# penghao-wu/vstar

Hardware: AMD Instinct MI355X
Metric: searched crops/sec (336x336 tiles, 7B VSM bf16) (higher is better)
Workload: dtype bf16; 1 GPU; BASELINE config 2: 32-crop batches/GPU, CLIP-ViT-L/14@336 (P=576) + LLaMA-7B prefill S=640 + OWL-ViT-B/16@768 + det/SAM heads, records all-gathered per step; seq_len=640, parallelism=dp1

## Files before the change

### include/vstar_hip.h

```cpp
#ifndef VSTAR_HIP_H
#define VSTAR_HIP_H

#include <stdint.h>
#include <stddef.h>

#ifdef __cplusplus
extern "C" {
#endif

#define VSTAR_ABI_VERSION 1

enum { VSTAR_F32 = 0, VSTAR_F16 = 1, VSTAR_BF16 = 2 };

enum {
  VSTAR_OK = 0,
  VSTAR_ERR_INVALID = -1,
  VSTAR_ERR_STATE = -2,
  VSTAR_ERR_MISSING = -3,
  VSTAR_ERR_HIP = -4,
  VSTAR_ERR_NOMEM = -5
};

typedef struct vstar_config {
  int32_t abi_version;
// ... 96 lines not shown
       VSTAR_EPI_NOSYNC = 0x100,
       VSTAR_EPI_TILE128 = 0x200,
       VSTAR_EPI_TILE256 = 0x400,
       VSTAR_EPI_TILE4W = 0x800    };

int vstar_op_gemm(void* stream, const uint16_t* dev_A, int64_t lda, const uint16_t* dev_W, const uint16_t* dev_bias,
                  const uint16_t* dev_residual, int64_t ldr, void* dev_C, int64_t ldc, int out_f32,
                  int M, int N, int K, int epilogue);
int vstar_op_gemm_norm(void* stream, const uint16_t* dev_A, int64_t lda, const uint16_t* dev_W, const uint16_t* dev_bias,
                       const uint16_t* dev_residual, int64_t ldr, void* dev_C, int64_t ldc, int M, int N, int K, int epilogue,
                       const float* dev_row_scale, float* dev_sumsq_out, int sumsq_ld);
int vstar_op_rms_rstd(void* stream, const uint16_t* dev_x, const float* dev_partials, int ld, int rows, int cols, float eps,
                      float* dev_r);
int vstar_op_ln_fold(void* stream, uint16_t* dev_W, uint16_t* dev_bias, const uint16_t* dev_g, const uint16_t* dev_b_ln,
                     int n_rows, int K);
int vstar_op_gemm_last_tile(void);
int vstar_op_gemm_plan(int M, int N, int K, int epilogue, int has_residual, int fused_rope, int cus);
int vstar_op_gemm_fp8(void* stream, const uint16_t* dev_A, const uint16_t* dev_W, const uint16_t* dev_bias,
                      const uint16_t* dev_residual, uint16_t* dev_C, int M, int N, int K, int epilogue, int iters, float* gemm_ms);
size_t vstar_op_mx_scale_bytes(int rows, int cols);
int64_t vstar_op_mx_scale_offset(int row, int k_block, int rows);
int vstar_op_quantize_mx(void* stream, const uint16_t* dev_X, uint8_t* dev_q, uint8_t* dev_scales, int rows, int cols);
int vstar_op_gemm_mx(void* stream, const uint8_t* dev_Aq, const uint8_t* dev_a_scales, const float* dev_row_scale, const uint16_t* dev_W,
                     const uint16_t* dev_residual, uint16_t* dev_C, uint8_t* dev_C8, uint8_t* dev_c_scales, float* dev_sumsq, int M, int N, int K,
                     int epilogue, int iters, float* gemm_ms);
int vstar_op_gemm_fp8_mxout(void* stream, const uint16_t* dev_A, const uint16_t* dev_W, uint8_t* dev_C8, uint8_t* dev_c_scales, int M, int N,
                            int K, int iters, float* gemm_ms);
int vstar_op_attention_mx(void* stream, const uint16_t* dev_qkv, uint8_t* dev_out8, uint8_t* dev_scales, int B, int S, int H);
int vstar_w8a8_mx_active(vstar_handle* h);
int vstar_op_layernorm(void* stream, const uint16_t* dev_x, const uint16_t* dev_gamma, const uint16_t* dev_beta,
// ... 47 lines not shown
```

### vstar_amd/_lib.py

```python
from __future__ import annotations

import ctypes
import os
from ctypes import POINTER, c_char_p, c_double, c_float, c_int, c_int32, c_int64, c_size_t, c_uint, c_uint16, c_void_p

from .config import CVqaConfig, CVstarConfig, MASK_RES, MAX_VERIFY, N_BOXES

LIB_PATH = os.environ.get("VSTAR_LIB") or os.path.join(os.path.dirname(os.path.abspath(__file__)), "libvstar_hip.so")

EXPORTS = [
    "vstar_create", "vstar_destroy", "vstar_last_error", "vstar_load_tensor", "vstar_finalize_weights",
    "vstar_vsm_score_batch", "vstar_upsample_mask", "vstar_debug_read", "vstar_stream", "vstar_profile_enable",
    "vstar_profile_read", "vstar_profile_read_fp8", "vstar_op_gemm", "vstar_op_layernorm", "vstar_op_rmsnorm", "vstar_op_attention",
    "vstar_op_attention_workspace", "vstar_image_set", "vstar_preprocess_crops", "vstar_heatmap_stats", "vstar_heatmap_stats_batch", "vstar_vsm_generate", "vstar_op_gemm_fp8",
    "vstar_op_gemm_last_tile", "vstar_op_gemm_plan", "vstar_op_gemm_norm", "vstar_op_rms_rstd", "vstar_op_ln_fold", "vstar_upsample_mask_ex", "vstar_vsm_score_grouped",
    "vstar_image_set_slot", "vstar_image_set_slot_async", "vstar_preprocess_crops_slots", "vstar_comm_unique_id", "vstar_comm_init", "vstar_allgather_results",
    "vstar_comm_destroy", "vstar_build_source_hash", "vstar_op_mx_scale_bytes", "vstar_op_mx_scale_offset", "vstar_op_quantize_mx",
    "vstar_op_gemm_mx", "vstar_op_gemm_fp8_mxout", "vstar_op_attention_mx", "vstar_w8a8_mx_active",
    "vstar_op_owl_class_logits", "vstar_op_owl_box_finish", "vstar_op_upsample2x_im2col3x3", "vstar_op_hyper_mask",
    "vstar_op_im2col_patch", "vstar_op_vit_assemble_tokens", "vstar_op_llm_embed_text", "vstar_op_add_bcast",
    "vstar_op_add_bcast_repeat", "vstar_op_bcast_rows", "vstar_op_owl_cls_mul", "vstar_op_gather_rows", "vstar_op_argmax_rows",
    "vstar_op_layernorm_ex", "vstar_op_rmsnorm_ex", "vstar_op_ln_rstd", "vstar_op_scale_cols", "vstar_op_fill",
    "vstar_op_quantize_rows_fp8", "vstar_op_rmsnorm_quant_fp8", "vstar_op_small_attention",
]

EXPORTS_VQA = [
    "vstar_vqa_create", "vstar_vqa_destroy", "vstar_vqa_last_error", "vstar_vqa_load_tensor", "vstar_vqa_finalize_weights",
    "vstar_vqa_encode_images", "vstar_vqa_forward", "vstar_vqa_debug_read", "vstar_vqa_last_forward_ms", "vstar_vqa_op_gemm",
    "vstar_vqa_forward_sample", "vstar_vqa_op_sample", "vstar_vqa_forward_beam", "vstar_vqa_kv_reorder", "vstar_vqa_kv_copy",
    "vstar_vqa_op_beam_select", "vstar_vqa_forward_score", "vstar_vqa_op_score",
# ... 105 lines not shown
    lib.vstar_profile_enable.restype = c_int
    lib.vstar_profile_read.argtypes = [H, POINTER(c_double), POINTER(c_int64), POINTER(c_double)]
    lib.vstar_profile_read.restype = c_int
    lib.vstar_profile_read_fp8.argtypes = [H, POINTER(c_double), POINTER(c_int64), POINTER(c_double)]
    lib.vstar_profile_read_fp8.restype = c_int
    lib.vstar_op_gemm.argtypes = [c_void_p, c_void_p, c_int64, c_void_p, c_void_p, c_void_p, c_int64, c_void_p, c_int64,
                                  c_int, c_int, c_int, c_int, c_int]
    lib.vstar_op_gemm.restype = c_int
    lib.vstar_op_gemm_norm.argtypes = [c_void_p, c_void_p, c_int64, c_void_p, c_void_p, c_void_p, c_int64, c_void_p, c_int64, c_int, c_int, c_int,
                                       c_int, c_void_p, c_void_p, c_int]
    lib.vstar_op_gemm_norm.restype = c_int
    lib.vstar_op_rms_rstd.argtypes = [c_void_p, c_void_p, c_void_p, c_int, c_int, c_int, c_float, c_void_p]
    lib.vstar_op_rms_rstd.restype = c_int
    lib.vstar_op_ln_fold.argtypes = [c_void_p, c_void_p, c_void_p, c_void_p, c_void_p, c_int, c_int]
    lib.vstar_op_ln_fold.restype = c_int
    lib.vstar_op_gemm_last_tile.argtypes = []
    lib.vstar_op_gemm_last_tile.restype = c_int
    lib.vstar_op_gemm_plan.argtypes = [c_int] * 7
    lib.vstar_op_gemm_plan.restype = c_int
    lib.vstar_op_gemm_fp8.argtypes = [c_void_p, c_void_p, c_void_p, c_void_p, c_void_p, c_void_p, c_int, c_int, c_int, c_int, c_int,
                                      POINTER(c_float)]
    lib.vstar_op_gemm_fp8.restype = c_int
    lib.vstar_op_mx_scale_bytes.argtypes = [c_int, c_int]
    lib.vstar_op_mx_scale_bytes.restype = c_size_t
    lib.vstar_op_mx_scale_offset.argtypes = [c_int, c_int, c_int]
    lib.vstar_op_mx_scale_offset.restype = ctypes.c_int64
    lib.vstar_op_quantize_mx.argtypes = [c_void_p, c_void_p, c_void_p, c_void_p, c_int, c_int]
    lib.vstar_op_quantize_mx.restype = c_int
    lib.vstar_op_gemm_mx.argtypes = [c_void_p] * 10 + [c_int, c_int, c_int, c_int, c_int, POINTER(c_float)]
    lib.vstar_op_gemm_mx.restype = c_int
# ... 111 lines not shown
```

### vstar_amd/csrc/engine.hip

```cpp
#include "llm_cached.hpp"
#include "mx.hpp"
#include <atomic>
#include <tuple>
#include <cstring>

namespace {
struct SamAttn { Lin q, k, v, out; int internal; };
struct SamLayer { SamAttn self_attn, t2i, i2t; lp_t *n1g, *n1b, *n2g, *n2b, *n3g, *n3b, *n4g, *n4b; Lin lin1, lin2; };
}

struct vstar_engine : EngineBase {
  vstar_config cfg{};
  VitTower clip, owl;
  Lin projector;
  lp_t* embed = nullptr;
  std::vector<LlmBlock> llm;
  lp_t* final_norm = nullptr;
  Lin lm_head;
  lp_t* rope = nullptr;
  Lin det0, det1, seg0, seg1;
  lp_t *owl_post_g = nullptr, *owl_post_b = nullptr, *owl_ln_g = nullptr, *owl_ln_b = nullptr;
  Lin cls_fused, box0, box1, box2;
  Lin vis_proj;
  lp_t *no_mask = nullptr, *dense_pe = nullptr, *iou_token = nullptr, *mask_tokens = nullptr;
// ... 17 lines not shown
  float *lr = nullptr, *lpart = nullptr;
  lp_t *lx = nullptr, *lh = nullptr, *lqkv = nullptr, *latt = nullptr, *lact = nullptr;
  lp_t* hsel = nullptr;
  lp_t *sel_att = nullptr, *sel_x = nullptr, *sel_h = nullptr, *sel_act = nullptr;
  float* vlogits = nullptr;
  lp_t *fc_tmp = nullptr, *emb_det = nullptr, *emb_seg = nullptr;
  int32_t *d_ids = nullptr, *d_rowidx = nullptr, *d_argmax = nullptr;
  lp_t *d_clip_pix = nullptr, *d_owl_pix = nullptr;
  lp_t *owl_feats_pre = nullptr, *owl_feats = nullptr, *box_t0 = nullptr, *box_t1 = nullptr;
  float *cls_emb = nullptr, *box_raw = nullptr;
  lp_t *s_src = nullptr, *s_keys = nullptr, *s_kpe = nullptr, *s_ia = nullptr, *s_ib = nullptr, *s_ic = nullptr;
  lp_t *s_tok0 = nullptr, *s_q = nullptr, *s_qpe = nullptr, *s_ta = nullptr, *s_tb = nullptr, *s_tc = nullptr, *s_td = nullptr,
         *s_mlp = nullptr;
  lp_t *s_col1 = nullptr, *s_c1 = nullptr, *s_c1n = nullptr, *s_col2 = nullptr, *s_c2 = nullptr, *s_hyp_in = nullptr,
         *s_hyp_a = nullptr, *s_hyp_b = nullptr, *s_hyper = nullptr;
  int32_t* d_tokidx = nullptr;
  vstar_result* d_results = nullptr;
  int last_B = 0, last_S = 0;
  void* d_stats = nullptr;
  void* d_stats_batch = nullptr; size_t stats_batch_cap = 0;
  void* comm = nullptr;
  float* d_up = nullptr; size_t up_cap = 0;
  struct ImageSlot { uint8_t* d = nullptr; size_t cap = 0; int H = 0, W = 0; };
  ImageSlot images[VSTAR_MAX_IMAGE_SLOTS];
  hipStream_t stream_up = nullptr;
  hipEvent_t ev_up[VSTAR_MAX_IMAGE_SLOTS] = {};
  std::atomic<int> up_pending[VSTAR_MAX_IMAGE_SLOTS] = {};
  uint8_t* h_stage[2] = {nullptr, nullptr};
  size_t stage_cap[2] = {0, 0};
  hipEvent_t ev_stage[2] = {nullptr, nullptr};
// ... 256 lines not shown
  RC(make_lin({"model.mask_decoder.output_upscaling.3.conv.weight"}, {"model.mask_decoder.output_upscaling.3.conv.bias"},
              &conv2, 64 * 9, nullptr, true));
  RC(make_lin({"model.mask_decoder.output_hypernetworks_mlps.0.layers.0.weight"},
              {"model.mask_decoder.output_hypernetworks_mlps.0.layers.0.bias"}, &hyp0, 256));
  RC(make_lin({"model.mask_decoder.output_hypernetworks_mlps.0.layers.1.weight"},
              {"model.mask_decoder.output_hypernetworks_mlps.0.layers.1.bias"}, &hyp1, 256));
  RC(make_lin({"model.mask_decoder.output_hypernetworks_mlps.0.layers.2.weight"},
              {"model.mask_decoder.output_hypernetworks_mlps.0.layers.2.bias"}, &hyp2, 256));
  if (conv1.N != 64 || conv2.N != 32 || hyp2.N != 32) { set_error("mask decoder dims"); return VSTAR_ERR_INVALID; }
  RC(dalloc(&s_src, prow * 256)); RC(dalloc(&s_keys, prow * 256)); RC(dalloc(&s_kpe, prow * 256));
  RC(dalloc(&s_ia, prow * 256)); RC(dalloc(&s_ib, prow * 256)); RC(dalloc(&s_ic, prow * 256));
  const size_t trow = (size_t)maxB * 6;
  RC(dalloc(&s_tok0, trow * 256)); RC(dalloc(&s_q, trow * 256)); RC(dalloc(&s_qpe, trow * 256));
  RC(dalloc(&s_ta, trow * 256)); RC(dalloc(&s_tb, trow * 256)); RC(dalloc(&s_tc, trow * 256)); RC(dalloc(&s_td, trow * 256));
  RC(dalloc(&s_mlp, trow * 2048));
  RC(dalloc(&s_col1, (size_t)maxB * 96 * 96 * 2304));
  RC(dalloc(&s_c1, (size_t)maxB * 96 * 96 * 64));
  RC(dalloc(&s_c1n, (size_t)maxB * 96 * 96 * 64));
  RC(dalloc(&s_col2, (size_t)maxB * 192 * 192 * 576));
  RC(dalloc(&s_c2, (size_t)maxB * 192 * 192 * 32));
  RC(dalloc(&s_hyp_in, (size_t)maxB * 256)); RC(dalloc(&s_hyp_a, (size_t)maxB * 256)); RC(dalloc(&s_hyp_b, (size_t)maxB * 256));
  RC(dalloc(&s_hyper, (size_t)maxB * 32));
  RC(dalloc(&d_tokidx, (size_t)maxB));
  {
    std::vector<int32_t> tix(maxB);
    for (int b = 0; b < maxB; ++b) tix[b] = b * 6 + 1;
    HIPCHK(hipMemcpy(d_tokidx, tix.data(), (size_t)maxB * 4, hipMemcpyHostToDevice));
  }
  RC(dalloc(&d_jobs, (size_t)maxB * 2));
  RC(dalloc(&d_lut, (size_t)3 * 256));
  {
    lp_t lut[3 * 256];
    clip_norm_lut(lut);
    HIPCHK(hipMemcpy(d_lut, lut, sizeof(lut), hipMemcpyHostToDevice));
  }
// ... 394 lines not shown
    RC(lin(s_q, 256, Ly.lin1, s_mlp, Ly.lin1.N, trow, VSTAR_EPI_RELU));
    RC(lin(s_mlp, Ly.lin1.N, Ly.lin2, s_tb, 256, trow, VSTAR_EPI_NONE, s_q, 256));
    KCHK(layernorm_lp(s_tb, Ly.n3g, Ly.n3b, s_q, trow, 256, 1e-5f, nullptr, 0, stream));
    KCHK(add_bcast(s_q, s_tok0, s_qpe, trow, 256, trow, stream));
    RC(sam_attn(Ly.i2t, s_kpe, NP, s_qpe, s_q, T, B, s_ia, s_ta, s_tb, s_ib, s_ic, s_keys));
    KCHK(layernorm_lp(s_ic, Ly.n4g, Ly.n4b, s_keys, prow, 256, 1e-5f, nullptr, 0, stream));
  }
  KCHK(add_bcast(s_q, s_tok0, s_qpe, trow, 256, trow, stream));
  KCHK(add_bcast(s_keys, dense_pe, s_kpe, prow, 256, NP, stream));
  RC(sam_attn(sam_final, s_qpe, T, s_kpe, s_keys, NP, B, s_ta, s_ia, s_ib, s_td, s_tb, s_q));
  KCHK(layernorm_lp(s_tb, sam_nfg, sam_nfb, s_q, trow, 256, 1e-5f, nullptr, 0, stream));
  KCHK(gather_rows(s_q, d_tokidx, s_hyp_in, B, 256, stream));
  RC(lin(s_hyp_in, 256, hyp0, s_hyp_a, 256, B, VSTAR_EPI_RELU));
  RC(lin(s_hyp_a, 256, hyp1, s_hyp_b, 256, B, VSTAR_EPI_RELU));
  RC(lin(s_hyp_b, 256, hyp2, s_hyper, 32, B));
  KCHK(upsample2x_im2col3x3(s_keys, s_col1, B, 48, 48, 256, stream));
  RC(lin(s_col1, 2304, conv1, s_c1, 64, B * 96 * 96));
  KCHK(layernorm_lp(s_c1, ln2d_g, ln2d_b, s_c1n, B * 96 * 96, 64, 1e-6f, nullptr, 1, stream));
  KCHK(upsample2x_im2col3x3(s_c1n, s_col2, B, 96, 96, 64, stream));
  RC(lin(s_col2, 576, conv2, s_c2, 32, B * 192 * 192, VSTAR_EPI_GELU));
  KCHK(hyper_mask(s_hyper, s_c2, res_f + offsetof(vstar_result, lowres_mask) / 4, rstride, B, 192 * 192, 32, stream));
  return 0;
}

int vstar_engine::finish_records(int nrec, int n_verify, unsigned flags, vstar_result* out) {
  if (n_verify > 0) {
    HIPCHK(hipMemcpy2DAsync((char*)d_results + offsetof(vstar_result, tf_argmax), sizeof(vstar_result), d_argmax,
                            (size_t)n_verify * 4, (size_t)n_verify * 4, nrec, hipMemcpyDeviceToDevice, stream));
  }
  if (out) {
    HIPCHK(hipMemcpyAsync(out, d_results, sizeof(vstar_result) * nrec,
                          (flags & VSTAR_F_DEVICE_OUTPUT) ? hipMemcpyDeviceToDevice : hipMemcpyDeviceToHost, stream));
  }
  if (!(flags & VSTAR_F_NO_SYNC)) {
    HIPCHK(hipStreamSynchronize(stream));
    collect_profile();
// ... 287 lines not shown
int vstar_create(const vstar_config* cfg, int device, vstar_handle** out) {
  if (!cfg || !out) { tls_error() = "null argument"; return VSTAR_ERR_INVALID; }
  if (cfg->abi_version != VSTAR_ABI_VERSION) { tls_error() = "ABI version mismatch"; return VSTAR_ERR_INVALID; }
  if (cfg->max_batch <= 0 || cfg->max_text_len < 2) { tls_error() = "bad limits"; return VSTAR_ERR_INVALID; }
  int n = 0;
  hipError_t e = hipGetDeviceCount(&n);
  if (e != hipSuccess || device < 0 || device >= n) {
    tls_error() = "no such HIP device (libvstar_hip has no CPU fallback)";
    return VSTAR_ERR_HIP;
  }
  vstar_engine* h = new vstar_engine();
  h->cfg = *cfg;
  if (const char* e = getenv("VSTAR_FUSED_ROPE")) h->fused_rope = atoi(e) != 0;
  if (const char* e = getenv("VSTAR_FOLD_NORMS")) h->fold_norms = atoi(e) != 0;
  if (const char* e = getenv("VSTAR_SCORE_GRAPH")) h->score_graph_on = atoi(e) != 0;
  h->device = device;
  if (hipSetDevice(device) != hipSuccess || hipStreamCreate(&h->stream) != hipSuccess) {
    tls_error() = "hipStreamCreate failed";
    delete h;
    return VSTAR_ERR_HIP;
  }
  if (const char* e = getenv("VSTAR_OWL_OVERLAP")) h->owl_overlap = atoi(e) != 0;
  if (hipStreamCreate(&h->stream2) != hipSuccess || hipEventCreateWithFlags(&h->ev_fork, hipEventDisableTiming) != hipSuccess ||
      hipEventCreateWithFlags(&h->ev_join, hipEventDisableTiming) != hipSuccess) {
    h->stream2 = nullptr;
  }
  if (hipStreamCreateWithFlags(&h->stream_up, hipStreamNonBlocking) != hipSuccess ||
      hipEventCreateWithFlags(&h->ev_stage[0], hipEventDisableTiming) != hipSuccess ||
      hipEventCreateWithFlags(&h->ev_stage[1], hipEventDisableTiming) != hipSuccess ||
      hipEventCreateWithFlags(&h->ev_pre, hipEventDisableTiming) != hipSuccess) {
// ... 217 lines not shown
  else if (n == "owl_pixels") { src = h->d_owl_pix; cnt = (int64_t)B * 3 * h->cfg.owl_image_size * h->cfg.owl_image_size; }
  else if (n == "clip_features") { src = h->clip.x; cnt = (int64_t)B * h->clip.N * h->clip.hidden; }
  else if (n == "llm_input") { src = h->lx; cnt = 0; }
  else if (n == "llm_hidden_loc") { src = h->hsel; cnt = (int64_t)B * h->cfg.llm_hidden; }
  else if (n == "embed_det") { src = h->emb_det; cnt = (int64_t)B * h->det1.N; }
  else if (n == "embed_seg") { src = h->emb_seg; cnt = (int64_t)B * 256; }
  else if (n == "owl_feats") { src = h->owl_feats; cnt = (int64_t)B * h->owl.P * h->owl.hidden; }
  else if (n == "sam_tokens") { src = h->s_q; cnt = (int64_t)B * 6 * 256; }
  else if (n == "sam_keys") { src = h->s_keys; cnt = (int64_t)B * h->owl.P * 256; }
  else if (n == "sam_src") { src = h->s_src; cnt = (int64_t)B * h->owl.P * 256; }
  else if (n == "sam_c1") { src = h->s_c1; cnt = (int64_t)B * 96 * 96 * 64; }
  else if (n == "sam_c1n") { src = h->s_c1n; cnt = (int64_t)B * 96 * 96 * 64; }
  else if (n == "sam_c2") { src = h->s_c2; cnt = (int64_t)B * 192 * 192 * 32; }
  else if (n == "sam_hyper") { src = h->s_hyper; cnt = (int64_t)B * 32; }
  else { h->set_error("unknown debug tensor: " + n); return VSTAR_ERR_INVALID; }
  if (cnt > cap) cnt = cap;
  std::vector<lp_t> tmp((size_t)cnt);
  if (hipStreamSynchronize(h->stream) != hipSuccess ||
      hipMemcpy(tmp.data(), src, (size_t)cnt * 2, hipMemcpyDeviceToHost) != hipSuccess) {
    h->set_error("debug_read: HIP failure");
    return VSTAR_ERR_HIP;
  }
  for (int64_t i = 0; i < cnt; ++i) out[i] = lp2f(tmp[(size_t)i]);
  return cnt;
}

void* vstar_stream(vstar_handle* h) { return h ? (void*)h->stream : nullptr; }

int vstar_profile_enable(vstar_handle* h, int on) {
  if (!h) return VSTAR_ERR_INVALID;
// ... 251 lines not shown

static int op_done(hipError_t e, void* stream) {
  if (e == hipSuccess) e = hipStreamSynchronize((hipStream_t)stream);
  return op_rc(e);
}
int vstar_op_owl_class_logits(void* stream, const float* emb, int ld, int Q, const uint16_t* query, float* out, int out_stride_crop,
                              int B, int rows_per_crop, int img_div) {
  return op_done(owl_class_logits(emb, ld, Q, query, out, out_stride_crop, B, rows_per_crop, (hipStream_t)stream, img_div), stream);
}
int vstar_op_owl_box_finish(void* stream, const float* raw, int ld, float* out, int out_stride_crop, int B, int grid, int img_div) {
  return op_done(owl_box_finish(raw, ld, out, out_stride_crop, B, grid, (hipStream_t)stream, img_div), stream);
}
int vstar_op_upsample2x_im2col3x3(void* stream, const uint16_t* src, uint16_t* A, int B, int h, int w, int C) {
  return op_done(upsample2x_im2col3x3(src, A, B, h, w, C, (hipStream_t)stream), stream);
}
int vstar_op_hyper_mask(void* stream, const uint16_t* hyper, const uint16_t* up, float* out, int out_stride_crop, int B, int npix,
                        int C) {
  return op_done(hyper_mask(hyper, up, out, out_stride_crop, B, npix, C, (hipStream_t)stream), stream);
}
int vstar_op_im2col_patch(void* stream, const uint16_t* pix, uint16_t* A, int B, int I, int ps, int Kpad) {
  return op_done(im2col_patch(pix, A, B, I, ps, Kpad, (hipStream_t)stream), stream);
}
int vstar_op_vit_assemble_tokens(void* stream, const uint16_t* patch, const uint16_t* cls, const uint16_t* pos, uint16_t* tokens,
                                 int B, int P, int C) {
  return op_done(vit_assemble_tokens(patch, cls, pos, tokens, B, P, C, (hipStream_t)stream), stream);
}
int vstar_op_llm_embed_text(void* stream, const int32_t* ids, int L, int img_col, int P, const uint16_t* table, int vocab,
                            uint16_t* x, int B, int C) {
  return op_done(llm_embed_text(ids, L, img_col, P, table, vocab, x, B, C, (hipStream_t)stream), stream);
}
// ... 58 lines not shown
```

### vstar_amd/csrc/heads.hip

```cpp
#include "common.hpp"
#include "kernels.hpp"

namespace VS_NS {

namespace {

__global__ __launch_bounds__(256) void owl_class_kernel(const float* __restrict__ emb, int ld, int Q,
                                                        const lp_t* __restrict__ query, float* __restrict__ out,
                                                        int out_stride_crop, int B, int rows_per_crop, int img_div) {
  const int lane = threadIdx.x & 63;
  const int64_t row = (int64_t)blockIdx.x * 4 + (threadIdx.x >> 6);
  if (row >= (int64_t)B * rows_per_crop) return;
  const int b = (int)(row / rows_per_crop), p = (int)(row % rows_per_crop);
  const float* er = emb + ((int64_t)(b / img_div) * rows_per_crop + p) * ld;
  const lp_t* qr = query + (int64_t)b * Q;
  float ee = 0.f, qq = 0.f;
  for (int d = lane; d < Q; d += 64) {
    const float e = rlp(er[d]), q = lp2f(qr[d]);
    ee += e * e;
    qq += q * q;
  }
  ee = wave_sum(ee);
  qq = wave_sum(qq);
  const float en = rlp(rlp(sqrtf(ee)) + 1e-6f), qn = rlp(rlp(sqrtf(qq)) + 1e-6f);
// ... 15 lines not shown
  const int64_t idx = (int64_t)blockIdx.x * blockDim.x + threadIdx.x;
  if (idx >= (int64_t)B * npatch * 4) return;
  const int c = (int)(idx & 3);
  const int64_t row = idx >> 2;
  const int p = (int)(row % npatch), b = (int)(row / npatch);
  float coord;
  if (c == 0) coord = (float)(p % grid + 1) / (float)grid;
  else if (c == 1) coord = (float)(p / grid + 1) / (float)grid;
  else coord = 1.0f / (float)grid;
  coord = fminf(fmaxf(coord, 0.f), 1.f);
  const float bias = logf(coord + 1e-4f) - log1pf(-coord + 1e-4f);
  const float v = rlp(rlp(raw[((int64_t)(b / img_div) * npatch + p) * ld + c]) + bias);
  out[(int64_t)b * out_stride_crop + p * 4 + c] = rlp(1.0f / (1.0f + __expf(-v)));
}

__global__ void up2x_im2col_kernel(const lp_t* __restrict__ src, lp_t* __restrict__ A, int B, int h, int w, int C) {
  const int cv = C >> 3;
  const int H2 = 2 * h, W2 = 2 * w;
  const int64_t idx = (int64_t)blockIdx.x * blockDim.x + threadIdx.x;
  const int64_t total = (int64_t)B * H2 * W2 * 9 * cv;
  if (idx >= total) return;
  const int v = (int)(idx % cv);
  int64_t r = idx / cv;
  const int tap = (int)(r % 9);
  r /= 9;
  const int X = (int)(r % W2);
  const int Y = (int)((r / W2) % H2);
  const int b = (int)(r / ((int64_t)W2 * H2));
  const int yy = Y + tap / 3 - 1, xx = X + tap % 3 - 1;
  lpx8 o = {0, 0, 0, 0, 0, 0, 0, 0};
  if (yy >= 0 && yy < H2 && xx >= 0 && xx < W2) {
    const float sy = fmaxf(0.5f * (yy + 0.5f) - 0.5f, 0.f), sx = fmaxf(0.5f * (xx + 0.5f) - 0.5f, 0.f);
    const int y0 = (int)sy, x0 = (int)sx;
    const int y1 = y0 + (y0 < h - 1 ? 1 : 0), x1 = x0 + (x0 < w - 1 ? 1 : 0);
    const float ly = sy - y0, lx = sx - x0;
    const lp_t* base = src + (int64_t)b * h * w * C + v * 8;
    const lpx8 v00 = *(const lpx8*)(base + ((int64_t)y0 * w + x0) * C);
    const lpx8 v01 = *(const lpx8*)(base + ((int64_t)y0 * w + x1) * C);
    const lpx8 v10 = *(const lpx8*)(base + ((int64_t)y1 * w + x0) * C);
    const lpx8 v11 = *(const lpx8*)(base + ((int64_t)y1 * w + x1) * C);
#pragma unroll
    for (int e = 0; e < 8; ++e) {
      const float t = (1.f - ly) * ((1.f - lx) * lp2f((lp_t)v00[e]) + lx * lp2f((lp_t)v01[e])) +
                      ly * ((1.f - lx) * lp2f((lp_t)v10[e]) + lx * lp2f((lp_t)v11[e]));
      o[e] = (short)f2lp(t);
    }
  }
  *(lpx8*)(A + idx * 8) = o;
}

template <int C>
__global__ void hyper_mask_kernel(const lp_t* __restrict__ hyper, const lp_t* __restrict__ up, float* __restrict__ out,
                                  int out_stride_crop, int B, int npix) {
  const int64_t idx = (int64_t)blockIdx.x * blockDim.x + threadIdx.x;
  if (idx >= (int64_t)B * npix) return;
  const int b = (int)(idx / npix), pix = (int)(idx % npix);
  const lp_t* u = up + idx * C;
  const lp_t* hy = hyper + (int64_t)b * C;
  float a = 0.f;
#pragma unroll
  for (int v = 0; v < C / 8; ++v) {
    const lpx8 x = *(const lpx8*)(u + v * 8);
    const lpx8 w = *(const lpx8*)(hy + v * 8);
#pragma unroll
    for (int e = 0; e < 8; ++e) a += lp2f((lp_t)x[e]) * lp2f((lp_t)w[e]);
  }
  out[(int64_t)b * out_stride_crop + pix] = rlp(a);
}

__global__ void resize_bilinear_kernel(const float* __restrict__ in, int hin, int win, float* __restrict__ out, int hout,
                                       int wout, float rh, float rw, int clamp_min0) {
  const int64_t idx = (int64_t)blockIdx.x * blockDim.x + threadIdx.x;
  if (idx >= (int64_t)hout * wout) return;
  const int x = (int)(idx % wout), y = (int)(idx / wout);
  const float sy = fmaxf(rh * (y + 0.5f) - 0.5f, 0.f), sx = fmaxf(rw * (x + 0.5f) - 0.5f, 0.f);
  const int y0 = (int)sy, x0 = (int)sx;
  const int y1 = y0 + (y0 < hin - 1 ? 1 : 0), x1 = x0 + (x0 < win - 1 ? 1 : 0);
  const float ly = sy - y0, lx = sx - x0;
  const float t = (1.f - ly) * ((1.f - lx) * in[y0 * win + x0] + lx * in[y0 * win + x1]) +
                  ly * ((1.f - lx) * in[y1 * win + x0] + lx * in[y1 * win + x1]);
  out[idx] = clamp_min0 ? fmaxf(t, 0.f) : t;
}
// ... 103 lines not shown
  return hipGetLastError();
}
hipError_t upsample2x_im2col3x3(const lp_t* src, lp_t* A, int B, int h, int w, int C, hipStream_t s) {
  if (C % 8) return hipErrorInvalidValue;
  hipLaunchKernelGGL(up2x_im2col_kernel, dim3(nblk((int64_t)B * 4 * h * w * 9 * (C / 8))), dim3(256), 0, s, src, A, B, h,
                     w, C);
  return hipGetLastError();
}
hipError_t hyper_mask(const lp_t* hyper, const lp_t* up, float* out, int out_stride_crop, int B, int npix, int C,
                      hipStream_t s) {
  if (C != 32) return hipErrorInvalidValue;
  hipLaunchKernelGGL(hyper_mask_kernel<32>, dim3(nblk((int64_t)B * npix)), dim3(256), 0, s, hyper, up, out,
                     out_stride_crop, B, npix);
  return hipGetLastError();
}
hipError_t resize_bilinear_clamp(const float* in, int hin, int win, float* out, int hout, int wout, hipStream_t s, int clamp_min0) {
  hipLaunchKernelGGL(resize_bilinear_kernel, dim3(nblk((int64_t)hout * wout)), dim3(256), 0, s, in, hin, win, out, hout,
                     wout, (float)hin / (float)hout, (float)win / (float)wout, clamp_min0);
  return hipGetLastError();
}

}
```

### vstar_amd/csrc/kernels.hpp

```cpp
#pragma once
#include <hip/hip_runtime.h>
#include <stdint.h>
#include <vector>
#include "../../include/vstar_hip.h"
#include "common.hpp"

namespace VS_NS {

struct GemmParams {
  const lp_t* A; int64_t lda; int a_group; int64_t a_gstride; int64_t a_off;
  const lp_t* W;
  const lp_t* bias;
  const lp_t* res; int64_t ldr;
  void* C; int64_t ldc; int c_group; int64_t c_gstride; int64_t c_off;
  int M, N, K;
  int debug_flags;
  const lp_t* norm_w; float norm_eps;
  const lp_t* rope_cs; int rope_S; int rope_cols;
  int rope_R0, rope_Lc;
  int rope_pos0, rope_tail;
  const float* a_scale; const float* w_scale;
  const float* row_scale; float* sumsq_out; int sumsq_ld;
  int stats_sum;
  int tile_force;
// ... 85 lines not shown
hipError_t llm_embed_text(const int32_t* ids, int L, int img_col, int P, const lp_t* table, int vocab, lp_t* x, int B,
                          int C, hipStream_t s);
hipError_t add_bcast(const lp_t* a, const lp_t* b, lp_t* out, int64_t rows, int cols, int64_t b_rows, hipStream_t s);
hipError_t add_bcast_repeat(const lp_t* a, const lp_t* b, lp_t* out, int n_out, int rep, int rows_per, int cols, hipStream_t s);
hipError_t bcast_rows(const lp_t* src, lp_t* dst, int nrep, int64_t rep_stride, int nrows, int cols, int64_t ld, hipStream_t s);
hipError_t owl_cls_mul(const lp_t* x, lp_t* y, int B, int N, int C, hipStream_t s);
hipError_t gather_rows(const lp_t* x, const int32_t* idx, lp_t* y, int rows, int cols, hipStream_t s);
hipError_t argmax_rows(const float* x, int rows, int cols, int ld, int32_t* out, int out_stride, hipStream_t s);

hipError_t owl_class_logits(const float* emb, int ld, int Q, const lp_t* query, float* out, int out_stride_crop,
                            int B, int rows_per_crop, hipStream_t s, int img_div = 1);
hipError_t owl_box_finish(const float* raw, int ld, float* out, int out_stride_crop, int B, int grid, hipStream_t s, int img_div = 1);
hipError_t upsample2x_im2col3x3(const lp_t* src, lp_t* A, int B, int h, int w, int C, hipStream_t s);
hipError_t hyper_mask(const lp_t* hyper, const lp_t* up, float* out, int out_stride_crop, int B, int npix, int C,
                      hipStream_t s);
hipError_t resize_bilinear_clamp(const float* in, int hin, int win, float* out, int hout, int wout, hipStream_t s, int clamp_min0 = 1);

hipError_t heat_stats_batch(const float* lowres, int hin, int win, const int* hw, const int* rects, const int* n_rects, int n,
                            int64_t max_pixels, double* out, unsigned* mm_scratch, hipStream_t s);

struct PreJob {
  int x0, y0, cw, ch;
  int in_w, in_h;
  int out;
  int hb_off, hc_off, hks;
  int vb_off, vc_off, vks;
  int img_w;
  int64_t temp_off;
  int64_t out_off;
  const uint8_t* img;
// ... 9 lines not shown
```

Measured before the change: 144.7 crops/s.

## Fuse SAM mask-head upsample, 3x3 conv, layernorm and hyper-mask into implicit-GEMM kernel

Replaces the upsample2x+im2col materialisation, the GEMM, the layernorm and the hyper_mask dot product with a single tiled kernel per conv stage. The kernel builds the upsampled patch in LDS, runs the 3x3 conv as an MFMA implicit GEMM, and applies bias/GELU, LN+GELU or the hypernetwork dot in the epilogue. This removes the very large col1/col2/c2 buffers and the global round-trips and launches between those steps. In exchange it adds complex LDS tiling, swizzles and bf16 rounding points that may differ slightly from the unfused path. It also adds an env flag and a debug path that rebuilds c2 on demand.

```diff
diff --git a/include/vstar_hip.h b/include/vstar_hip.h
--- a/include/vstar_hip.h
+++ b/include/vstar_hip.h
@@ -134,6 +134,9 @@
                       float* dev_r);
 int vstar_op_ln_fold(void* stream, uint16_t* dev_W, uint16_t* dev_bias, const uint16_t* dev_g, const uint16_t* dev_b_ln,
                      int n_rows, int K);
+int vstar_op_upconv3x3(void* stream, const uint16_t* dev_src, const uint16_t* dev_W, const uint16_t* dev_bias, uint16_t* dev_out,
+                       const uint16_t* dev_hyper, float* dev_mask, int mask_stride_crop, const uint16_t* dev_ln_g,
+                       const uint16_t* dev_ln_b, uint16_t* dev_out_ln, float ln_eps, int B, int h, int w, int C, int N, int epilogue);
 int vstar_op_gemm_last_tile(void);
 int vstar_op_gemm_plan(int M, int N, int K, int epilogue, int has_residual, int fused_rope, int cus);
 int vstar_op_gemm_fp8(void* stream, const uint16_t* dev_A, const uint16_t* dev_W, const uint16_t* dev_bias,
diff --git a/vstar_amd/_lib.py b/vstar_amd/_lib.py
--- a/vstar_amd/_lib.py
+++ b/vstar_amd/_lib.py
@@ -13,7 +13,7 @@
     "vstar_vsm_score_batch", "vstar_upsample_mask", "vstar_debug_read", "vstar_stream", "vstar_profile_enable",
     "vstar_profile_read", "vstar_profile_read_fp8", "vstar_op_gemm", "vstar_op_layernorm", "vstar_op_rmsnorm", "vstar_op_attention",
     "vstar_op_attention_workspace", "vstar_image_set", "vstar_preprocess_crops", "vstar_heatmap_stats", "vstar_heatmap_stats_batch", "vstar_vsm_generate", "vstar_op_gemm_fp8",
-    "vstar_op_gemm_last_tile", "vstar_op_gemm_plan", "vstar_op_gemm_norm", "vstar_op_rms_rstd", "vstar_op_ln_fold", "vstar_upsample_mask_ex", "vstar_vsm_score_grouped",
+    "vstar_op_gemm_last_tile", "vstar_op_gemm_plan", "vstar_op_gemm_norm", "vstar_op_rms_rstd", "vstar_op_ln_fold", "vstar_op_upconv3x3", "vstar_upsample_mask_ex", "vstar_vsm_score_grouped",
     "vstar_image_set_slot", "vstar_image_set_slot_async", "vstar_preprocess_crops_slots", "vstar_comm_unique_id", "vstar_comm_init", "vstar_allgather_results",
     "vstar_comm_destroy", "vstar_build_source_hash", "vstar_op_mx_scale_bytes", "vstar_op_mx_scale_offset", "vstar_op_quantize_mx",
     "vstar_op_gemm_mx", "vstar_op_gemm_fp8_mxout", "vstar_op_attention_mx", "vstar_w8a8_mx_active",
@@ -149,6 +149,8 @@
     lib.vstar_op_rms_rstd.restype = c_int
     lib.vstar_op_ln_fold.argtypes = [c_void_p, c_void_p, c_void_p, c_void_p, c_void_p, c_int, c_int]
     lib.vstar_op_ln_fold.restype = c_int
+    lib.vstar_op_upconv3x3.argtypes = [c_void_p] * 7 + [c_int] + [c_void_p] * 3 + [c_float] + [c_int] * 6
+    lib.vstar_op_upconv3x3.restype = c_int
     lib.vstar_op_gemm_last_tile.argtypes = []
     lib.vstar_op_gemm_last_tile.restype = c_int
     lib.vstar_op_gemm_plan.argtypes = [c_int] * 7
diff --git a/vstar_amd/csrc/engine.hip b/vstar_amd/csrc/engine.hip
--- a/vstar_amd/csrc/engine.hip
+++ b/vstar_amd/csrc/engine.hip
@@ -55,6 +55,8 @@
          *s_mlp = nullptr;
   lp_t *s_col1 = nullptr, *s_c1 = nullptr, *s_c1n = nullptr, *s_col2 = nullptr, *s_c2 = nullptr, *s_hyp_in = nullptr,
          *s_hyp_a = nullptr, *s_hyp_b = nullptr, *s_hyper = nullptr;
+  bool fused_upconv = true;
+  int materialise_c2(int B);
   int32_t* d_tokidx = nullptr;
   vstar_result* d_results = nullptr;
   int last_B = 0, last_S = 0;
@@ -341,11 +343,13 @@
   RC(dalloc(&s_tok0, trow * 256)); RC(dalloc(&s_q, trow * 256)); RC(dalloc(&s_qpe, trow * 256));
   RC(dalloc(&s_ta, trow * 256)); RC(dalloc(&s_tb, trow * 256)); RC(dalloc(&s_tc, trow * 256)); RC(dalloc(&s_td, trow * 256));
   RC(dalloc(&s_mlp, trow * 2048));
-  RC(dalloc(&s_col1, (size_t)maxB * 96 * 96 * 2304));
   RC(dalloc(&s_c1, (size_t)maxB * 96 * 96 * 64));
   RC(dalloc(&s_c1n, (size_t)maxB * 96 * 96 * 64));
-  RC(dalloc(&s_col2, (size_t)maxB * 192 * 192 * 576));
-  RC(dalloc(&s_c2, (size_t)maxB * 192 * 192 * 32));
+  if (!fused_upconv) {
+    RC(dalloc(&s_col1, (size_t)maxB * 96 * 96 * 2304));
+    RC(dalloc(&s_col2, (size_t)maxB * 192 * 192 * 576));
+    RC(dalloc(&s_c2, (size_t)maxB * 192 * 192 * 32));
+  }
   RC(dalloc(&s_hyp_in, (size_t)maxB * 256)); RC(dalloc(&s_hyp_a, (size_t)maxB * 256)); RC(dalloc(&s_hyp_b, (size_t)maxB * 256));
   RC(dalloc(&s_hyper, (size_t)maxB * 32));
   RC(dalloc(&d_tokidx, (size_t)maxB));
@@ -770,12 +774,27 @@
   RC(lin(s_hyp_in, 256, hyp0, s_hyp_a, 256, B, VSTAR_EPI_RELU));
   RC(lin(s_hyp_a, 256, hyp1, s_hyp_b, 256, B, VSTAR_EPI_RELU));
   RC(lin(s_hyp_b, 256, hyp2, s_hyper, 32, B));
+  float* lowres = res_f + offsetof(vstar_result, lowres_mask) / 4;
+  if (fused_upconv) {
+    KCHK(upconv3x3(s_keys, conv1.W, conv1.b, s_c1, nullptr, nullptr, 0, ln2d_g, ln2d_b, s_c1n, 1e-6f, B, 48, 48, 256, 64,
+                   VSTAR_EPI_NONE, stream));
+    KCHK(upconv3x3(s_c1n, conv2.W, conv2.b, nullptr, s_hyper, lowres, rstride, nullptr, nullptr, nullptr, 0.f, B, 96, 96, 64, 32,
+                   VSTAR_EPI_GELU, stream));
+    return 0;
+  }
   KCHK(upsample2x_im2col3x3(s_keys, s_col1, B, 48, 48, 256, stream));
   RC(lin(s_col1, 2304, conv1, s_c1, 64, B * 96 * 96));
   KCHK(layernorm_lp(s_c1, ln2d_g, ln2d_b, s_c1n, B * 96 * 96, 64, 1e-6f, nullptr, 1, stream));
   KCHK(upsample2x_im2col3x3(s_c1n, s_col2, B, 96, 96, 64, stream));
   RC(lin(s_col2, 576, conv2, s_c2, 32, B * 192 * 192, VSTAR_EPI_GELU));
-  KCHK(hyper_mask(s_hyper, s_c2, res_f + offsetof(vstar_result, lowres_mask) / 4, rstride, B, 192 * 192, 32, stream));
+  KCHK(hyper_mask(s_hyper, s_c2, lowres, rstride, B, 192 * 192, 32, stream));
+  return 0;
+}
+
+int vstar_engine::materialise_c2(int B) {
+  if (!s_c2) RC(dalloc(&s_c2, (size_t)cfg.max_batch * 192 * 192 * 32));
+  KCHK(upconv3x3(s_c1n, conv2.W, conv2.b, s_c2, nullptr, nullptr, 0, nullptr, nullptr, nullptr, 0.f, B, 96, 96, 64, 32, VSTAR_EPI_GELU,
+                 stream));
   return 0;
 }
 
@@ -1093,6 +1112,7 @@
   if (const char* e = getenv("VSTAR_FUSED_ROPE")) h->fused_rope = atoi(e) != 0;
   if (const char* e = getenv("VSTAR_FOLD_NORMS")) h->fold_norms = atoi(e) != 0;
   if (const char* e = getenv("VSTAR_SCORE_GRAPH")) h->score_graph_on = atoi(e) != 0;
+  if (const char* e = getenv("VSTAR_FUSED_UPCONV")) h->fused_upconv = atoi(e) != 0;
   h->device = device;
   if (hipSetDevice(device) != hipSuccess || hipStreamCreate(&h->stream) != hipSuccess) {
     tls_error() = "hipStreamCreate failed";
@@ -1340,6 +1360,10 @@
   else if (n == "sam_c2") { src = h->s_c2; cnt = (int64_t)B * 192 * 192 * 32; }
   else if (n == "sam_hyper") { src = h->s_hyper; cnt = (int64_t)B * 32; }
   else { h->set_error("unknown debug tensor: " + n); return VSTAR_ERR_INVALID; }
+  if (n == "sam_c2" && h->fused_upconv) {
+    if (int rc = h->materialise_c2(B)) return rc;
+    src = h->s_c2;
+  }
   if (cnt > cap) cnt = cap;
   std::vector<lp_t> tmp((size_t)cnt);
   if (hipStreamSynchronize(h->stream) != hipSuccess ||
@@ -1621,6 +1645,12 @@
 int vstar_op_upsample2x_im2col3x3(void* stream, const uint16_t* src, uint16_t* A, int B, int h, int w, int C) {
   return op_done(upsample2x_im2col3x3(src, A, B, h, w, C, (hipStream_t)stream), stream);
 }
+int vstar_op_upconv3x3(void* stream, const uint16_t* src, const uint16_t* W, const uint16_t* bias, uint16_t* out, const uint16_t* hyper,
+                       float* mask, int mask_stride_crop, const uint16_t* ln_g, const uint16_t* ln_b, uint16_t* out_ln, float ln_eps,
+                       int B, int h, int w, int C, int N, int epilogue) {
+  return op_done(upconv3x3(src, W, bias, out, hyper, mask, mask_stride_crop, ln_g, ln_b, out_ln, ln_eps, B, h, w, C, N, epilogue,
+                           (hipStream_t)stream), stream);
+}
 int vstar_op_hyper_mask(void* stream, const uint16_t* hyper, const uint16_t* up, float* out, int out_stride_crop, int B, int npix,
                         int C) {
   return op_done(hyper_mask(hyper, up, out, out_stride_crop, B, npix, C, (hipStream_t)stream), stream);
diff --git a/vstar_amd/csrc/heads.hip b/vstar_amd/csrc/heads.hip
--- a/vstar_amd/csrc/heads.hip
+++ b/vstar_amd/csrc/heads.hip
@@ -1,5 +1,6 @@
 #include "common.hpp"
 #include "kernels.hpp"
+#include "gemm_epilogue.hpp"
 
 namespace VS_NS {
 
@@ -53,6 +54,43 @@
   out[(int64_t)b * out_stride_crop + p * 4 + c] = rlp(1.0f / (1.0f + __expf(-v)));
 }
 
+struct Up2xTaps { lpx8 v00, v01, v10, v11; float ly, lx; bool inside; };
+__device__ __forceinline__ Up2xTaps up2x_taps(const lp_t* __restrict__ img, int h, int w, int C, int yy, int xx, int v) {
+  Up2xTaps t;
+  t.v00 = t.v01 = t.v10 = t.v11 = (lpx8){0, 0, 0, 0, 0, 0, 0, 0};
+  t.ly = t.lx = 0.f;
+  t.inside = yy >= 0 && yy < 2 * h && xx >= 0 && xx < 2 * w;
+  if (t.inside) {
+    const float sy = fmaxf(0.5f * (yy + 0.5f) - 0.5f, 0.f), sx = fmaxf(0.5f * (xx + 0.5f) - 0.5f, 0.f);
+    const int y0 = (int)sy, x0 = (int)sx;
+    const int y1 = y0 + (y0 < h - 1 ? 1 : 0), x1 = x0 + (x0 < w - 1 ? 1 : 0);
+    t.ly = sy - y0;
+    t.lx = sx - x0;
+    const lp_t* base = img + v * 8;
+    t.v00 = *(const lpx8*)(base + ((int64_t)y0 * w + x0) * C);
+    t.v01 = *(const lpx8*)(base + ((int64_t)y0 * w + x1) * C);
+    t.v10 = *(const lpx8*)(base + ((int64_t)y1 * w + x0) * C);
+    t.v11 = *(const lpx8*)(base + ((int64_t)y1 * w + x1) * C);
+  }
+  return t;
+}
+__device__ __forceinline__ lpx8 up2x_blend(const Up2xTaps& t) {
+  lpx8 o = {0, 0, 0, 0, 0, 0, 0, 0};
+  if (t.inside) {
+    const float ly = t.ly, lx = t.lx;
+#pragma unroll
+    for (int e = 0; e < 8; ++e) {
+      const float r = (1.f - ly) * ((1.f - lx) * lp2f((lp_t)t.v00[e]) + lx * lp2f((lp_t)t.v01[e])) +
+                      ly * ((1.f - lx) * lp2f((lp_t)t.v10[e]) + lx * lp2f((lp_t)t.v11[e]));
+      o[e] = (short)f2lp(r);
+    }
+  }
+  return o;
+}
+__device__ __forceinline__ lpx8 up2x_pixel8(const lp_t* __restrict__ img, int h, int w, int C, int yy, int xx, int v) {
+  return up2x_blend(up2x_taps(img, h, w, C, yy, xx, v));
+}
+
 __global__ void up2x_im2col_kernel(const lp_t* __restrict__ src, lp_t* __restrict__ A, int B, int h, int w, int C) {
   const int cv = C >> 3;
   const int H2 = 2 * h, W2 = 2 * w;
@@ -66,45 +104,216 @@
   const int X = (int)(r % W2);
   const int Y = (int)((r / W2) % H2);
   const int b = (int)(r / ((int64_t)W2 * H2));
-  const int yy = Y + tap / 3 - 1, xx = X + tap % 3 - 1;
-  lpx8 o = {0, 0, 0, 0, 0, 0, 0, 0};
-  if (yy >= 0 && yy < H2 && xx >= 0 && xx < W2) {
-    const float sy = fmaxf(0.5f * (yy + 0.5f) - 0.5f, 0.f), sx = fmaxf(0.5f * (xx + 0.5f) - 0.5f, 0.f);
-    const int y0 = (int)sy, x0 = (int)sx;
-    const int y1 = y0 + (y0 < h - 1 ? 1 : 0), x1 = x0 + (x0 < w - 1 ? 1 : 0);
-    const float ly = sy - y0, lx = sx - x0;
-    const lp_t* base = src + (int64_t)b * h * w * C + v * 8;
-    const lpx8 v00 = *(const lpx8*)(base + ((int64_t)y0 * w + x0) * C);
-    const lpx8 v01 = *(const lpx8*)(base + ((int64_t)y0 * w + x1) * C);
-    const lpx8 v10 = *(const lpx8*)(base + ((int64_t)y1 * w + x0) * C);
-    const lpx8 v11 = *(const lpx8*)(base + ((int64_t)y1 * w + x1) * C);
-#pragma unroll
-    for (int e = 0; e < 8; ++e) {
-      const float t = (1.f - ly) * ((1.f - lx) * lp2f((lp_t)v00[e]) + lx * lp2f((lp_t)v01[e])) +
-                      ly * ((1.f - lx) * lp2f((lp_t)v10[e]) + lx * lp2f((lp_t)v11[e]));
-      o[e] = (short)f2lp(t);
-    }
-  }
-  *(lpx8*)(A + idx * 8) = o;
-}
-
+  *(lpx8*)(A + idx * 8) = up2x_pixel8(src + (int64_t)b * h * w * C, h, w, C, Y + tap / 3 - 1, X + tap % 3 - 1, v);
+}
+
+template <int C>
+__device__ __forceinline__ float hyper_dot(const lp_t* u, const lp_t* __restrict__ hy) {
+  float a = 0.f;
+#pragma unroll
+  for (int v = 0; v < C / 8; ++v) {
+    const lpx8 x = *(const lpx8*)(u + v * 8);
+    const lpx8 w = *(const lpx8*)(hy + v * 8);
+#pragma unroll
+    for (int e = 0; e < 8; ++e) a += lp2f((lp_t)x[e]) * lp2f((lp_t)w[e]);
+  }
+  return rlp(a);
+}
 template <int C>
 __global__ void hyper_mask_kernel(const lp_t* __restrict__ hyper, const lp_t* __restrict__ up, float* __restrict__ out,
                                   int out_stride_crop, int B, int npix) {
   const int64_t idx = (int64_t)blockIdx.x * blockDim.x + threadIdx.x;
   if (idx >= (int64_t)B * npix) return;
   const int b = (int)(idx / npix), pix = (int)(idx % npix);
-  const lp_t* u = up + idx * C;
-  const lp_t* hy = hyper + (int64_t)b * C;
-  float a = 0.f;
-#pragma unroll
-  for (int v = 0; v < C / 8; ++v) {
-    const lpx8 x = *(const lpx8*)(u + v * 8);
-    const lpx8 w = *(const lpx8*)(hy + v * 8);
-#pragma unroll
-    for (int e = 0; e < 8; ++e) a += lp2f((lp_t)x[e]) * lp2f((lp_t)w[e]);
-  }
-  out[(int64_t)b * out_stride_crop + pix] = rlp(a);
+  out[(int64_t)b * out_stride_crop + pix] = hyper_dot<C>(up + idx * C, hyper + (int64_t)b * C);
+}
+
+template <int C, int N>
+struct UpconvCfg {
+  static constexpr int TH = C >= 256 ? 8 : 16, TW = 16, PW = TW + 2;
+  static constexpr int NPOS = (TH + 2) * PW;
+  static constexpr int PATCH_BYTES = NPOS * C * 2;
+  static constexpr int NS = 9 * C / 64;
+  static constexpr int SLICE_BYTES = N * 128;
+  static constexpr bool RES = NS * SLICE_BYTES <= 40 * 1024;
+  static constexpr int W_BYTES = (RES ? NS : 2) * SLICE_BYTES;
+  static constexpr int OROW = N * 2 + 16;
+  static constexpr int LDS_BYTES = PATCH_BYTES + W_BYTES;
+  static_assert(TH * TW * OROW <= PATCH_BYTES, "the epilogue image reuses the patch");
+};
+
+template <int C>
+__device__ __forceinline__ int upconv_swz(int pos) { return C >= 128 ? (pos & 15) : ((pos >> 1) & (C / 8 - 1)); }
+
+template <int C, int N, int EPI>
+__global__ __launch_bounds__(256) void upconv3x3_kernel(const lp_t* __restrict__ src, const lp_t* __restrict__ W,
+                                                        const lp_t* __restrict__ bias, lp_t* __restrict__ out,
+                                                        const lp_t* __restrict__ hyper, float* __restrict__ mask,
+                                                        int mask_stride, const lp_t* __restrict__ ln_g,
+                                                        const lp_t* __restrict__ ln_b, lp_t* __restrict__ out_ln, int ln_cols,
+                                                        float ln_eps, int B, int h, int w) {
+  using G = UpconvCfg<C, N>;
+  constexpr int TH = G::TH, TW = G::TW, PW = G::PW, MF = TH / 4, NF = N / 16, CV = C / 8, K = 9 * C;
+  static_assert(C % 64 == 0 && N % 16 == 0 && TH % 4 == 0, "tile shape");
+  extern __shared__ __attribute__((aligned(16))) char smem[];
+  char* patch = smem;
+  char* wlds = smem + G::PATCH_BYTES;
+  const int tid = threadIdx.x, lane = tid & 63;
+  const int wave = __builtin_amdgcn_readfirstlane(tid >> 6);
+  const int H2 = 2 * h, W2 = 2 * w;
+  const int tiles_x = (W2 + TW - 1) / TW, tiles_y = (H2 + TH - 1) / TH;
+  const int b = blockIdx.x / (tiles_x * tiles_y);
+  const int trem = blockIdx.x - b * (tiles_x * tiles_y);
+  const int ty0 = (trem / tiles_x) * TH, tx0 = (trem % tiles_x) * TW;
+
+  constexpr int WCH = N * 8 / 256;
+  static_assert(N * 8 % 256 == 0, "W slice chunks per thread");
+  auto w_load = [&](int ks, lpx8 (&r)[WCH]) {
+#pragma unroll
+    for (int i = 0; i < WCH; ++i) {
+      const int q = i * 256 + tid;
+      r[i] = *(const lpx8*)(W + (int64_t)(q >> 3) * K + ks * 64 + (q & 7) * 8);
+    }
+  };
+  auto w_store = [&](int slot, const lpx8 (&r)[WCH]) {
+#pragma unroll
+    for (int i = 0; i < WCH; ++i) {
+      const int q = i * 256 + tid, row = q >> 3;
+      *(lpx8*)(wlds + slot * G::SLICE_BYTES + row * 128 + (((q & 7) ^ ((row >> 1) & 7)) * 16)) = r[i];
+    }
+  };
+  {
+    constexpr int NL = G::RES ? G::NS : 1;
+    lpx8 r[NL][WCH];
+#pragma unroll
+    for (int ks = 0; ks < NL; ++ks) w_load(ks, r[ks]);
+#pragma unroll
+    for (int ks = 0; ks < NL; ++ks) w_store(ks, r[ks]);
+  }
+  const lp_t* img = src + (int64_t)b * h * w * C;
+  constexpr int SU = 4;
+  for (int it0 = tid; it0 < G::NPOS * CV; it0 += 256 * SU) {
+    Up2xTaps taps[SU];
+#pragma unroll
+    for (int u = 0; u < SU; ++u) {
+      const int it = it0 + u * 256, pos = it / CV;
+      const int py = pos / PW, px = pos - py * PW;
+      taps[u] = up2x_taps(img, h, w, C, it < G::NPOS * CV ? ty0 + py - 1 : -1, tx0 + px - 1, it % CV);
+    }
+#pragma unroll
+    for (int u = 0; u < SU; ++u) {
+      const int it = it0 + u * 256, pos = it / CV;
+      if (it < G::NPOS * CV) *(lpx8*)(patch + pos * (C * 2) + (((it % CV) ^ upconv_swz<C>(pos)) * 16)) = up2x_blend(taps[u]);
+    }
+  }
+  __syncthreads();
+
+  const int fr = lane & 15, fq = lane >> 4;
+  f32x4 acc[MF][NF];
+#pragma unroll
+  for (int m = 0; m < MF; ++m)
+#pragma unroll
+    for (int n = 0; n < NF; ++n) acc[m][n] = (f32x4){0.f, 0.f, 0.f, 0.f};
+  const int wswz = (fr >> 1) & 7;
+#pragma unroll 1
+  for (int ks = 0; ks < G::NS; ++ks) {
+    lpx8 pre[WCH];
+    if constexpr (!G::RES) { if (ks + 1 < G::NS) w_load(ks + 1, pre); }
+    const int tap = ks * 64 / C, cc0 = (ks * 64 % C) / 8;
+    const int ky = tap / 3, kx = tap - ky * 3;
+    const char* wb = wlds + (G::RES ? ks : (ks & 1)) * G::SLICE_BYTES;
+#pragma unroll
+    for (int kk = 0; kk < 2; ++kk) {
+      lpx8 af[MF], wf[NF];
+#pragma unroll
+      for (int m = 0; m < MF; ++m) {
+        const int pos = (wave * MF + m + ky) * PW + fr + kx;
+        af[m] = *(const lpx8*)(patch + pos * (C * 2) + (((cc0 + kk * 4 + fq) ^ upconv_swz<C>(pos)) * 16));
+      }
+#pragma unroll
+      for (int n = 0; n < NF; ++n) wf[n] = *(const lpx8*)(wb + (n * 16 + fr) * 128 + (((kk * 4 + fq) ^ wswz) * 16));
+#pragma unroll
+      for (int m = 0; m < MF; ++m)
+#pragma unroll
+        for (int n = 0; n < NF; ++n) acc[m][n] = mfma_16x16x32(wf[n], af[m], acc[m][n]);
+    }
+    if constexpr (!G::RES) {
+      if (ks + 1 < G::NS) w_store((ks + 1) & 1, pre);
+      __syncthreads();
+    }
+  }
+
+  GemmParams p{};
+  p.bias = bias; p.C = out; p.ldc = N; p.N = N;
+  if (out) {
+#pragma unroll
+    for (int m = 0; m < MF; ++m) {
+      const int Y = ty0 + wave * MF + m, X = tx0 + fr;
+      if (Y >= H2 || X >= W2) continue;
+      const int64_t crow = ((int64_t)b * H2 + Y) * W2 + X;
+#pragma unroll
+      for (int n = 0; n < NF; ++n) gemm_epilogue_store<EPI, false>(p, crow, n * 16 + fq * 4, N, acc[m][n], acc[m][n]);
+    }
+  }
+  if (mask || out_ln) {
+    if constexpr (G::RES) __syncthreads();
+#pragma unroll
+    for (int m = 0; m < MF; ++m)
+#pragma unroll
+      for (int n = 0; n < NF; ++n) {
+        float o[4];
+        gemm_epilogue_values<EPI, false>(p, n * 16 + fq * 4, N, acc[m][n], acc[m][n], o);
+        const lpx4 v = {(short)f2lp(o[0]), (short)f2lp(o[1]), (short)f2lp(o[2]), (short)f2lp(o[3])};
+        *(lpx4*)(patch + ((wave * MF + m) * 16 + fr) * G::OROW + (n * 16 + fq * 4) * 2) = v;
+      }
+    __syncthreads();
+  }
+  if (mask) {
+    for (int pix = tid; pix < TH * TW; pix += 256) {
+      const int Y = ty0 + pix / TW, X = tx0 + pix % TW;
+      if (Y < H2 && X < W2)
+        mask[(int64_t)b * mask_stride + (int64_t)Y * W2 + X] = hyper_dot<N>((const lp_t*)(patch + pix * G::OROW), hyper + (int64_t)b * N);
+    }
+  }
+  if (out_ln) {
+    constexpr int LPP = N / 8;
+    static_assert(TH * TW * LPP % 256 == 0 && (LPP & (LPP - 1)) == 0, "whole passes: the shuffles need every lane");
+    for (int it = tid; it < TH * TW * LPP; it += 256) {
+      const int pix = it / LPP, j = it % LPP;
+      const lpx8 t = *(const lpx8*)(patch + pix * G::OROW + j * 16);
+      float v[8], sum = 0.f;
+#pragma unroll
+      for (int e = 0; e < 8; ++e) {
+        v[e] = lp2f((lp_t)t[e]);
+        sum += v[e];
+      }
+      sum += 0.f;
+#pragma unroll
+      for (int o = LPP / 2; o > 0; o >>= 1) sum += __shfl_xor(sum, o, 64);
+      const float mean = sum / (float)ln_cols;
+      float sq = 0.f;
+#pragma unroll
+      for (int e = 0; e < 8; ++e) {
+        const float d = v[e] - mean;
+        sq += d * d;
+      }
+      sq += 0.f;
+#pragma unroll
+      for (int o = LPP / 2; o > 0; o >>= 1) sq += __shfl_xor(sq, o, 64);
+      const float rstd = rsqrtf(sq / (float)ln_cols + ln_eps);
+      const lpx8 g = *(const lpx8*)(ln_g + j * 8);
+      const lpx8 bb = *(const lpx8*)(ln_b + j * 8);
+      lpx8 o8;
+#pragma unroll
+      for (int e = 0; e < 8; ++e) {
+        float r = (v[e] - mean) * rstd * lp2f((lp_t)g[e]) + lp2f((lp_t)bb[e]);
+        r = act_gelu_erf(rlp(r));
+        o8[e] = (short)f2lp(r);
+      }
+      const int Y = ty0 + pix / TW, X = tx0 + pix % TW;
+      if (Y < H2 && X < W2) *(lpx8*)(out_ln + (((int64_t)b * H2 + Y) * W2 + X) * N + j * 8) = o8;
+    }
+  }
 }
 
 __global__ void resize_bilinear_kernel(const float* __restrict__ in, int hin, int win, float* __restrict__ out, int hout,
@@ -238,6 +447,37 @@
                      out_stride_crop, B, npix);
   return hipGetLastError();
 }
+namespace {
+template <int C, int N, int EPI>
+hipError_t upconv3x3_launch(const lp_t* src, const lp_t* W, const lp_t* bias, lp_t* out, const lp_t* hyper, float* mask,
+                            int mask_stride, const lp_t* ln_g, const lp_t* ln_b, lp_t* out_ln, float ln_eps, int B, int h, int w,
+                            hipStream_t s) {
+  using G = UpconvCfg<C, N>;
+  auto kern = upconv3x3_kernel<C, N, EPI>;
+  static bool attr_done = false;
+  if (!attr_done) {
+    const hipError_t e = hipFuncSetAttribute((const void*)kern, hipFuncAttributeMaxDynamicSharedMemorySize, G::LDS_BYTES);
+    if (e != hipSuccess) return e;
+    attr_done = true;
+  }
+  const int64_t tiles = (int64_t)B * ((2 * h + G::TH - 1) / G::TH) * ((2 * w + G::TW - 1) / G::TW);
+  if (tiles > 0x7fffffff) return hipErrorInvalidValue;
+  hipLaunchKernelGGL(kern, dim3((unsigned)tiles), dim3(256), G::LDS_BYTES, s, src, W, bias, out, hyper, mask, mask_stride, ln_g, ln_b,
+                     out_ln, N, ln_eps, B, h, w);
+  return hipGetLastError();
+}
+}
+hipError_t upconv3x3(const lp_t* src, const lp_t* W, const lp_t* bias, lp_t* out, const lp_t* hyper, float* mask, int mask_stride,
+                     const lp_t* ln_g, const lp_t* ln_b, lp_t* out_ln, float ln_eps, int B, int h, int w, int C, int N, int epilogue,
+                     hipStream_t s) {
+  if (B <= 0 || h <= 0 || w <= 0) return hipSuccess;
+  if ((!out && !mask && !out_ln) || (mask && (!hyper || N != 32)) || (out_ln && (!ln_g || !ln_b))) return hipErrorInvalidValue;
+  if (C == 256 && N == 64 && epilogue == VSTAR_EPI_NONE)
+    return upconv3x3_launch<256, 64, VSTAR_EPI_NONE>(src, W, bias, out, hyper, mask, mask_stride, ln_g, ln_b, out_ln, ln_eps, B, h, w, s);
+  if (C == 64 && N == 32 && epilogue == VSTAR_EPI_GELU)
+    return upconv3x3_launch<64, 32, VSTAR_EPI_GELU>(src, W, bias, out, hyper, mask, mask_stride, ln_g, ln_b, out_ln, ln_eps, B, h, w, s);
+  return hipErrorInvalidValue;
+}
 hipError_t resize_bilinear_clamp(const float* in, int hin, int win, float* out, int hout, int wout, hipStream_t s, int clamp_min0) {
   hipLaunchKernelGGL(resize_bilinear_kernel, dim3(nblk((int64_t)hout * wout)), dim3(256), 0, s, in, hin, win, out, hout,
                      wout, (float)hin / (float)hout, (float)win / (float)wout, clamp_min0);
diff --git a/vstar_amd/csrc/kernels.hpp b/vstar_amd/csrc/kernels.hpp
--- a/vstar_amd/csrc/kernels.hpp
+++ b/vstar_amd/csrc/kernels.hpp
@@ -123,6 +123,9 @@
 hipError_t upsample2x_im2col3x3(const lp_t* src, lp_t* A, int B, int h, int w, int C, hipStream_t s);
 hipError_t hyper_mask(const lp_t* hyper, const lp_t* up, float* out, int out_stride_crop, int B, int npix, int C,
                       hipStream_t s);
+hipError_t upconv3x3(const lp_t* src, const lp_t* W, const lp_t* bias, lp_t* out, const lp_t* hyper, float* mask, int mask_stride,
+                     const lp_t* ln_g, const lp_t* ln_b, lp_t* out_ln, float ln_eps, int B, int h, int w, int C, int N, int epilogue,
+                     hipStream_t s);
 hipError_t resize_bilinear_clamp(const float* in, int hin, int win, float* out, int hout, int wout, hipStream_t s, int clamp_min0 = 1);
 
 hipError_t heat_stats_batch(const float* lowres, int hin, int win, const int* hw, const int* rects, const int* n_rects, int n,
```

Result: no change. 145.8 crops/s (median of 6 runs) (+0.8%).
